# jgaeddert/liquid-usrp

Measured on AMD Instinct MI355X. Metric: complex Msamples/s through multichannelrx, higher is better.
Workload: dtype f32

## Files before the change

liquid-usrp_amd/csrc/ofdmsync.hip:

```cpp
#include "devmath.h"
#include "kernels.h"
#include <utility>

namespace mcrx {

#define WV 64
#ifndef SY_PART
#define SY_PART -1
#endif
#ifndef SY_PROFILE
#define SY_PROFILE 0
#endif
#ifndef H128_EARLY_OUT
#define H128_EARLY_OUT 1
#endif
#ifndef SY_RANK
#define SY_RANK 1
#endif
#ifndef SY_SEG_BURST
#define SY_SEG_BURST 1
#endif
#define SY_PROF(a) (SY_PROFILE && ((a).debug & 2) != 0)
#ifdef MCRX_DEVEL
#define MCRX_DEVEL_ABLATE(a) ((unsigned)(a).debug >> 8 << 6)
// ... 2386 lines not shown
    const int64_t t_ev0 = job->s.cur + (int64_t)job->s.timer - 1;
    const int64_t ws0 = t_ev0 - L + 1 + cb;
    uint32_t dth = uni(job->s.nco_dtheta);
    uint32_t th_ws = uni(job->s.nco_theta_ref + (uint32_t)(ws0 - job->s.nco_t_ref) * job->s.nco_dtheta);
    uint32_t pc = uni(job->s.pilot_count);
    float phi_prime = job->s.phi_prime, p1_prime = job->s.p1_prime;
    int32_t r_ws = (int32_t)uni((uint32_t)(ws0 - a.buf_first));
    const float2 *chb = a.chan + ((size_t)a.chan_off + ch) * MCRX_TILE_S;
    const size_t tstride = (size_t)a.chan_stride * MCRX_TILE_S;
    uint8_t *soft = a.jsoft + (size_t)jj * 8 * c.max_enc_len;
    float2 *syms = reinterpret_cast<float2 *>(a.sarena + job->syms_off);
    const bool soft_mode = c.payload_soft != 0;
    uint32_t nmax = 0;
#pragma unroll
    for (int k = 0; k < FR; k++) {
        const uint32_t v = (uint32_t)__builtin_amdgcn_readlane((int)(active ? nsym : 0u), k * G);
        nmax = v > nmax ? v : nmax;
    }
    const int32_t r_max = (int32_t)(a.end - a.buf_first) - 1;

    auto load_win = [&](int32_t rw, float2 (&x)[E]) {
#pragma unroll
        for (int e = 0; e < E; e++) {
            int32_t r = rw + i + G * e;
            r = r < 0 ? 0 : (r > r_max ? r_max : r);
            x[e] = chb[(size_t)(r >> MCRX_TILE_SH) * tstride + (size_t)(r & (MCRX_TILE_S - 1))];
        }
    };
    float2 cur[E], nxt[E];
    load_win(r_ws, cur);
    uint32_t psi = 0;
    for (uint32_t n = 0; n < nmax; n++) {
        const bool live = active && n < nsym;
        load_win(r_ws + L, nxt);
#pragma unroll
        for (int e = 0; e < E; e++) cur[e] = rot_down(cur[e], u32rev(th_ws + (uint32_t)(i + G * e) * dth));
#pragma unroll
        for (int J = E / 2; J >= 1; J >>= 1) {
#pragma unroll
            for (int e = 0; e < E; e++) {
                if ((e & J) == 0) {
                    const float2 u = cur[e], v = cur[e + J];
                    const float rev = (float)((i + G * e) & (G * J - 1)) * (0.5f / (float)(G * J));
                    cur[e] = cadd(u, v); cur[e + J] = rot_down(csub(u, v), rev);
                }
            }
        }
#define SY_QSTAGE(ST, H)                                                                           \
        if constexpr (H < G) {                                                                     \
            _Pragma("unroll") for (int e = 0; e < E; e++) {                                        \
                const float sx = bfly_leg<H>(cur[e].x, sgc[ST]), sy = bfly_leg<H>(cur[e].y, sgc[ST]);  \
                if (H == 1) cur[e] = make_float2(sx, sy);                                          \
                else cur[e] = make_float2(sx * twc[ST].x - sy * twc[ST].y, sx * twc[ST].y + sy * twc[ST].x); \
            }                                                                                      \
        }
        SY_QSTAGE(0, 32) SY_QSTAGE(1, 16) SY_QSTAGE(2, 8) SY_QSTAGE(3, 4) SY_QSTAGE(4, 2) SY_QSTAGE(5, 1)
#undef SY_QSTAGE
#pragma unroll
        for (int e = 0; e < E; e++) {
            cur[e] = cmul(cur[e], R[e]);
            if (pr[e] >= 0) qpil[16 * g + pr[e]] = cur[e];
        }
        wave_sync_lds();
        float2 P = qpil[16 * g + (i < Mp ? i : 0)];
        uint32_t pi_ = pc + (uint32_t)(i < 16 ? i : 0); pi_ = pi_ >= 255u ? pi_ - 255u : pi_;
        const bool pneg = pseq[pi_ < 255u ? pi_ : 0u] == 0;
        wave_sync_lds();
        if (pneg) { P.x = -P.x; P.y = -P.y; }
        const float v = atan2_fast(P.y, P.x);
        const float prev = dpp_mov<0x111, false>(v, v);
        const float turns = rintf((v - prev) * 0.15915494309189535f);
        const float y = fmaf(-TWO_PI_F, row_scan_fast(turns), v);
        const float p0 = group_total(row_scan_fast(pf0 * y));
        float p1 = group_total(row_scan_fast(pf1 * y));
        pc += (uint32_t)Mp; pc = pc >= 255u ? pc - 255u : pc;
        p1 = 0.3f * p1 + (1.0f - 0.3f) * p1_prime;
        p1_prime = p1;
        const float p0r = p0 * 0.15915494309189535f;
        const bool full = (psi + (uint32_t)Md) * bps <= nbits;
        float2 Z[E];
#pragma unroll
        for (int e = 0; e < E; e++) Z[e] = rot_down(cur[e], fmaf(p1, fxr[e], p0r));
        unsigned long long pending = __ballot(live);
        while (pending) {
            const int src = __builtin_ctzll(pending);
            const uint32_t umod = (uint32_t)__builtin_amdgcn_readlane((int)mod, src), ubps = (uint32_t)__builtin_amdgcn_readlane((int)bps, src);
            const bool sel = live && mod == umod;
            pending &= ~__ballot(sel);
            const uint8_t *unbt = reinterpret_cast<const uint8_t *>(umod == 27 ? qnb16 : qnb64);
#pragma unroll
            for (int e = 0; e < E; e++) {
                const uint32_t idx = psi + (uint32_t)dr[e];
                const bool ok = sel && dr[e] >= 0 && idx < mod_len;
                uint8_t sb[6];
                const unsigned hs = demod_soft(unbt, umod, Z[e], sb);
                if (!soft_mode) {
#pragma unroll
                    for (int kb = 0; kb < 6; kb++) sb[kb] = (uint8_t)(((hs >> ((ubps - 1 - kb) & 7)) & 1) ? 255 : 0);
                }
                if (!ok) continue;
                syms[idx] = Z[e];
                uint8_t *dst = soft + (size_t)idx * ubps;
                if (full) {
                    if (ubps == 2)      *reinterpret_cast<uint16_t *>(dst) = (uint16_t)(sb[0] | (sb[1] << 8));
                    else if (ubps == 1) dst[0] = sb[0];
                    else {
                        *reinterpret_cast<uint16_t *>(dst) = (uint16_t)(sb[0] | (sb[1] << 8));
                        *reinterpret_cast<uint16_t *>(dst + 2) = (uint16_t)(sb[2] | (sb[3] << 8));
                        if (ubps == 6) *reinterpret_cast<uint16_t *>(dst + 4) = (uint16_t)(sb[4] | (sb[5] << 8));
                    }
                } else {
                    for (unsigned kb = 0; kb < ubps; kb++) if (idx * ubps + kb < nbits) dst[kb] = sb[kb];
                }
            }
        }
        psi += (uint32_t)Md;
        float dphi = p0 - phi_prime;
        dphi -= TWO_PI_F * rintf(dphi * 0.15915494309189535f);
        phi_prime = p0;
        const uint32_t dnew = dth + uni((uint32_t)__float2int_rn(dphi * (1e-3f * 683565275.5764316f)));
        th_ws += (uint32_t)(L - cb) * dth + (uint32_t)cb * dnew;
        if (live) dth = dnew;
        r_ws += L;
#pragma unroll
        for (int e = 0; e < E; e++) cur[e] = nxt[e];
    }
    if (i == 0 && active) a.jobs[j].s.nco_dtheta = dth;
}

#include "payload_lean.hpp"

#define DK_T 256
#ifndef DK_FUSED
#define DK_FUSED 1
#endif
#ifndef DK_NT_LOAD
#define DK_NT_LOAD 1
#endif
extern __shared__ __attribute__((aligned(16))) unsigned long long dk_soft[];
#define DKP(e) ((e) ^ (((e) >> 5) & 31u))
__device__ __forceinline__ unsigned il_cols_below(unsigned s0, unsigned len, unsigned Ncol, unsigned rem)
{
    auto span = [&](unsigned a0, unsigned b0) { const unsigned lo = a0 < rem ? a0 : rem, hi = b0 < rem ? b0 : rem; return hi - lo; };
    return (s0 + len <= Ncol) ? span(s0, s0 + len) : span(s0, Ncol) + span(0u, s0 + len - Ncol);
}
__device__ __forceinline__ void divmod_small(unsigned a, unsigned b, unsigned &q, unsigned &r)
{
    q = (unsigned)((float)a * __builtin_amdgcn_rcpf((float)b));
    int rr = (int)a - (int)(q * b);
    if (rr < 0) { q--; rr += (int)b; }
    if (rr >= (int)b) { q++; rr -= (int)b; }
    r = (unsigned)rr;
}
__device__ void il_pass_lds(unsigned n, unsigned Mi, unsigned Ncol, unsigned mask, unsigned dummy)
{
    const unsigned n2 = n / 2, c0 = n / 3;
    unsigned long long m64 = 0;
#pragma unroll
    for (int k = 0; k < 8; k++) if ((mask >> (7 - k)) & 1) m64 |= 0xFFull << (8 * k);
    unsigned R, rem, cnt0 = 0, t0, s1, c0r;
    divmod_small(n2, Ncol, R, rem);
    if (c0 < n2) divmod_small(n2 - c0 + Ncol - 1, Ncol, cnt0, t0);
    divmod_small(c0, Ncol, t0, c0r);
    s1 = c0r + 1; s1 -= s1 >= Ncol ? Ncol : 0u;
    const unsigned sa = s1 < rem ? rem - s1 : 0u, sb = Ncol - (s1 > rem ? s1 : rem), sw = rem < s1 ? rem : s1;
    const unsigned B1 = sa * (R + 1), B2 = B1 + sb * R, B3 = B2 + sw * (R + 1);
    constexpr int UN = 4;
    for (unsigned i0 = threadIdx.x; i0 < n2; i0 += UN * DK_T) {
        unsigned ea[UN], eb[UN];
        unsigned long long va[UN], vb[UN];
#pragma unroll
        for (int u = 0; u < UN; u++) {
            const unsigned i = i0 + u * DK_T;
            const unsigned ip = i - cnt0;
            const bool g1 = ip < B1, g2 = ip < B2, g3 = ip < B3;
            unsigned d = (g1 || (!g2 && g3)) ? R + 1 : R;
            d = d ? d : 1u;
            const unsigned off = g1 ? ip : g2 ? ip - B1 : g3 ? ip - B2 : ip - B3;
            const unsigned lbase = g1 ? 0u : g2 ? sa : g3 ? sa + sb : sa + sb + sw;
            unsigned q, m; divmod_small(off, d, q, m);
            const unsigned len = lbase + q;
            unsigned cm = s1 + len; cm -= cm >= Ncol ? Ncol : 0u;
            const bool first = i < cnt0;
            const unsigned j = first ? i * Ncol + c0 : m * Ncol + cm;
            const bool ok = i < n2 && j < n2 && (first || (len < Ncol && m < Mi));
            ea[u] = ok ? DKP(2 * i) : dummy;
            eb[u] = ok ? DKP(2 * j + 1) : dummy;
            va[u] = dk_soft[ea[u]]; vb[u] = dk_soft[eb[u]];
        }
#pragma unroll
        for (int u = 0; u < UN; u++) {
            dk_soft[ea[u]] = (va[u] & ~m64) | (vb[u] & m64);
            dk_soft[eb[u]] = (vb[u] & ~m64) | (va[u] & m64);
        }
    }
    __syncthreads();
}
__device__ uint32_t crc32_tree(const CodingDev cod, uint32_t tab_off, uint32_t msg_off, uint32_t n)
{
    const uint32_t *lds_tab = reinterpret_cast<const uint32_t *>(reinterpret_cast<const uint8_t *>(dk_soft) + tab_off);
    const uint8_t *p = reinterpret_cast<const uint8_t *>(dk_soft) + msg_off;
    const int r = lane_id();
    uint32_t C = 1, lc = 0;
    while (64u * C < n) { C <<= 1; lc++; }
    const int64_t hi = (int64_t)n - (int64_t)r * C, lo0 = hi - (int64_t)C;
    const int64_t lo = lo0 < 0 ? 0 : lo0;
    const uint32_t rmax = n ? (n + C - 1) / C - 1 : 0;
    uint32_t s = ((uint32_t)r == rmax) ? 0xFFFFFFFFu : 0u;
    for (int64_t i = lo; i < hi; i++) s = (s >> 8) ^ lds_tab[(s ^ p[i]) & 0xff];
#pragma unroll
    for (int k = 0; k < 6; k++) {
        const uint32_t v = (uint32_t)__shfl_down((int)s, 1 << k, WV);
        if ((r & ((2 << k) - 1)) == 0 && r + (1 << k) < WV) {
            const uint32_t *A = cod.crc_zadv + (size_t)(lc + k) * 1024;
            s ^= A[v & 0xff] ^ A[256 + ((v >> 8) & 0xff)] ^ A[512 + ((v >> 16) & 0xff)] ^ A[768 + (v >> 24)];
        }
    }
    return ~(uint32_t)__shfl((int)s, 0, WV);
}
__device__ __forceinline__ void decode_frame(SyncArgs &a, const uint32_t j, uint32_t lds_soft_bytes, uint32_t msg_bytes)
{
    const uint32_t ch = a.jobs[j].ch;
    if (ch >= a.nch || a.jobs[j].arena_off == ~0ull) return;
    const SyncConsts &c = a.c;
    const uint32_t n_msg = a.jobs[j].s.payload_len, crc = a.jobs[j].s.check, fec0 = a.jobs[j].s.fec0, fec1 = a.jobs[j].s.fec1;
    const uint32_t e1 = a.jobs[j].s.enc_len;
    uint8_t *soft = a.jsoft + (size_t)j * 8 * c.max_enc_len;
    const uint32_t crc_len = (crc == 6) ? 4u : 0u, n0 = n_msg + crc_len;
    const bool prof = SY_PROF(a) && j == 7;
    long long tk[8]; int ntk = 0;
#define DK_TICK() if (prof) tk[ntk++] = (long long)__builtin_readcyclecounter();
    DK_TICK()
    const bool lds_path = c.payload_soft && fec0 == 1 && (fec1 == 6 || fec1 == 7 || fec1 == 1) && 8u * e1 <= lds_soft_bytes && !(a.no_fast & 8);
    if (!lds_path) {
        const uint32_t moff = (c.il_off && e1 < c.il_n) ? c.il_off[e1] : ~0u;
        const bool conv_pre = c.payload_soft && fec1 == 11 && a.vit_scratch && moff != ~0u && 8u * e1 <= lds_soft_bytes && !(a.no_fast & 8) &&
                              vf::rows_for(8u * fec_enc_len_d(fec0, n0) + 6u) <= a.vit_rows;
        const bool conv_go = conv_pre;
        if (c.payload_soft && fec1 == 11 && !a.vit_scratch && a.hint && threadIdx.x == 0) a.hint[HINT_K7_SEEN] = 1u;
        if (conv_go) {
            const unsigned long long *g64 = reinterpret_cast<const unsigned long long *>(soft);
            for (uint32_t i = threadIdx.x; i < e1; i += DK_T) dk_soft[DKP(i)] = g64[i];
            __syncthreads();
            const uint4 *mp = reinterpret_cast<const uint4 *>(c.il_map + (size_t)moff * 8);
            const uint8_t *sb = reinterpret_cast<const uint8_t *>(dk_soft);
            unsigned long long *o64 = reinterpret_cast<unsigned long long *>(soft);
            for (uint32_t i = threadIdx.x; i < e1; i += DK_T) {
                const uint4 m = mp[i];
                const uint32_t lo = (uint32_t)sb[m.x & 0xffffu] | ((uint32_t)sb[m.x >> 16] << 8) | ((uint32_t)sb[m.y & 0xffffu] << 16) | ((uint32_t)sb[m.y >> 16] << 24);
                const uint32_t hi = (uint32_t)sb[m.z & 0xffffu] | ((uint32_t)sb[m.z >> 16] << 8) | ((uint32_t)sb[m.w & 0xffffu] << 16) | ((uint32_t)sb[m.w >> 16] << 24);
                o64[i] = (unsigned long long)lo | ((unsigned long long)hi << 32);
            }
        }
        if (threadIdx.x == 0 && a.gen_list) {
            uint32_t *gl = as_global(a.gen_list);
            uint32_t tag = j;
            if (conv_go) {
                tag |= 0x80000000u;
            }
            gl[1u + atomicAdd(gl, 1u)] = tag;
        }
        return;
    }
    if (lds_path) {
        const uint32_t moff_h = (fec1 == 6 && c.il_off && e1 < c.il_n) ? c.il_off[e1] : ~0u;
        const bool fused = DK_FUSED && moff_h != ~0u;
        constexpr int SU = 4;
        const uint2 *mp2 = reinterpret_cast<const uint2 *>(c.il_map + (size_t)(fused ? moff_h : 0u) * 8);
        uint2 pm[SU][3];
        if (fused) {
#pragma unroll
            for (int u = 0; u < SU; u++) {
                const uint32_t i = threadIdx.x + u * DK_T, ii = i < n0 ? i : 0u;
#pragma unroll
                for (int k = 0; k < 3; k++) pm[u][k] = mp2[3u * ii + k];
            }
        }
        const unsigned long long *g64 = reinterpret_cast<const unsigned long long *>(soft);
        for (uint32_t b0 = 0; b0 < e1; b0 += 8 * DK_T) {
            unsigned long long v[8];
#pragma unroll
#if DK_NT_LOAD
            for (int u = 0; u < 8; u++) { const uint32_t i = b0 + u * DK_T + threadIdx.x; v[u] = __builtin_nontemporal_load(g64 + (i < e1 ? i : 0)); }
#else
            for (int u = 0; u < 8; u++) { const uint32_t i = b0 + u * DK_T + threadIdx.x; v[u] = g64[i < e1 ? i : 0]; }
#endif
#pragma unroll
            for (int u = 0; u < 8; u++) { const uint32_t i = b0 + u * DK_T + threadIdx.x; if (i < e1) dk_soft[DKP(i)] = v[u]; }
        }
        __syncthreads();
        DK_TICK()
        unsigned long long *cur = dk_soft;
        uint8_t *msg = reinterpret_cast<uint8_t *>(dk_soft) + 2 * lds_soft_bytes;
        if (fused) {
            const uint8_t *sb = reinterpret_cast<const uint8_t *>(dk_soft);
            for (uint32_t b0 = 0; b0 < n0; b0 += SU * DK_T) {
                if (b0) {
#pragma unroll
                    for (int u = 0; u < SU; u++) {
                        const uint32_t i = b0 + threadIdx.x + u * DK_T, ii = i < n0 ? i : 0u;
#pragma unroll
                        for (int k = 0; k < 3; k++) pm[u][k] = mp2[3u * ii + k];
                    }
                }
#pragma unroll
                for (int u = 0; u < SU; u++) {
                    const uint32_t i = b0 + threadIdx.x + u * DK_T;
                    if (i >= n0) break;
                    uint32_t w[3];
#pragma unroll
                    for (int k = 0; k < 3; k++) {
                        const uint2 m = pm[u][k];
                        w[k] = (uint32_t)sb[m.x & 0xffffu] | ((uint32_t)sb[m.x >> 16] << 8) | ((uint32_t)sb[m.y & 0xffffu] << 16) | ((uint32_t)sb[m.y >> 16] << 24);
                    }
                    msg[i] = (uint8_t)h128_dec_soft_words(w[0], w[1], w[2]);
                }
            }
        } else if (fec1 != 1) {
            const uint32_t moff = (c.il_off && e1 < c.il_n) ? c.il_off[e1] : ~0u;
            if (moff != ~0u) {
                const uint4 *mp = reinterpret_cast<const uint4 *>(c.il_map + (size_t)moff * 8);
                const uint8_t *sb = reinterpret_cast<const uint8_t *>(dk_soft);
                unsigned long long *dst = dk_soft + lds_soft_bytes / 8;
                for (uint32_t i0 = threadIdx.x; i0 < e1; i0 += 8 * DK_T) {
                    uint4 mm[8];
#pragma unroll
                    for (int u = 0; u < 8; u++) { const uint32_t i = i0 + u * DK_T; mm[u] = mp[i < e1 ? i : 0]; }
#pragma unroll
                    for (int u = 0; u < 8; u++) {
                        const uint32_t i = i0 + u * DK_T;
                        if (i >= e1) break;
                        const uint4 m = mm[u];
                        const uint32_t lo = (uint32_t)sb[m.x & 0xffffu] | ((uint32_t)sb[m.x >> 16] << 8) | ((uint32_t)sb[m.y & 0xffffu] << 16) | ((uint32_t)sb[m.y >> 16] << 24);
                        const uint32_t hi = (uint32_t)sb[m.z & 0xffffu] | ((uint32_t)sb[m.z >> 16] << 8) | ((uint32_t)sb[m.w & 0xffffu] << 16) | ((uint32_t)sb[m.w >> 16] << 24);
                        dst[DKP(i)] = (unsigned long long)lo | ((unsigned long long)hi << 32);
                    }
                }
                cur = dst;
                __syncthreads();
            } else {
                unsigned Mi, Ni; il_dims(e1, Mi, Ni);
                const unsigned dummy = 2 * (lds_soft_bytes / 8) + msg_bytes / 8;
                il_pass_lds(e1, Mi, Ni + 8, 0x33, dummy);
                il_pass_lds(e1, Mi, Ni + 4, 0x55, dummy);
                il_pass_lds(e1, Mi, Ni + 2, 0x0f, dummy);
                il_pass_lds(e1, Mi, Ni, 0xff, dummy);
            }
        }
        DK_TICK()
        const uint32_t *w32 = reinterpret_cast<const uint32_t *>(cur);
        auto word = [&](uint32_t w) { return w32[2u * DKP(w >> 1) + (w & 1u)]; };
        auto slice = [&](uint32_t g) -> unsigned {
            const unsigned long long v = cur[DKP(g)];
            unsigned b = 0;
#pragma unroll
            for (int kb = 0; kb < 8; kb++) b = (b << 1) | ((((unsigned)(v >> (8 * kb)) & 0xffu) > 127u) ? 1u : 0u);
            return b;
        };
        if (fused) {
        } else if (fec1 == 6) {
            for (uint32_t i = threadIdx.x; i < n0; i += DK_T) msg[i] = (uint8_t)h128_dec_soft_words(word(3 * i), word(3 * i + 1), word(3 * i + 2));
        } else if (fec1 == 7) {
            const uint32_t G = n0 / 3, rr = n0 % 3;
            for (uint32_t g = threadIdx.x; g < G; g += DK_T) {
                const unsigned s0 = golay_dec_sym((slice(6 * g) << 16) | (slice(6 * g + 1) << 8) | slice(6 * g + 2));
                const unsigned s1 = golay_dec_sym((slice(6 * g + 3) << 16) | (slice(6 * g + 4) << 8) | slice(6 * g + 5));
                msg[3 * g]     = (uint8_t)((s0 >> 4) & 0xff);
                msg[3 * g + 1] = (uint8_t)(((s0 << 4) & 0xf0) | ((s1 >> 8) & 0x0f));
                msg[3 * g + 2] = (uint8_t)(s1 & 0xff);
            }
            if (threadIdx.x < rr) {
                const uint32_t b = 6 * G + 3 * threadIdx.x;
                msg[3 * G + threadIdx.x] = (uint8_t)(golay_dec_sym((slice(b) << 16) | (slice(b + 1) << 8) | slice(b + 2)) & 0xff);
            }
        } else {
            for (uint32_t i = threadIdx.x; i < n0; i += DK_T) msg[i] = (uint8_t)slice(i);
        }
        __syncthreads();
        DK_TICK()
        {
            uint32_t *dst = reinterpret_cast<uint32_t *>(a.arena + a.jobs[j].arena_off);
            const uint32_t *src = reinterpret_cast<const uint32_t *>(msg);
            for (uint32_t i = threadIdx.x; i < (n_msg + 3) / 4; i += DK_T) dst[i] = src[i];
        }
        const bool by_pos = crc_len && c.crc_pos && n_msg >= 4 && n_msg <= c.crc_pos_n;
        if (by_pos) {
            uint32_t acc = 0;
            for (uint32_t i0 = threadIdx.x; i0 < n_msg; i0 += 8 * DK_T) {
                uint32_t t[8];
#pragma unroll
                for (int u = 0; u < 8; u++) {
                    const uint32_t i = i0 + u * DK_T, ii = i < n_msg ? i : n_msg - 1;
                    const uint32_t b = (uint32_t)msg[ii] ^ (ii < 4 ? 0xffu : 0u);
                    t[u] = c.crc_pos[(size_t)(n_msg - 1 - ii) * 256 + b];
                }
#pragma unroll
                for (int u = 0; u < 8; u++) if (i0 + u * DK_T < n_msg) acc ^= t[u];
            }
            acc = wave_xor_u32(acc);
            if ((threadIdx.x & (WV - 1)) == 0) reinterpret_cast<uint32_t *>(dk_soft)[256 + threadIdx.x / WV] = acc;
        }
        reinterpret_cast<uint32_t *>(dk_soft)[threadIdx.x] = c.cod.crc_byte[threadIdx.x];
        __syncthreads();
        if (threadIdx.x >= WV) return;
    }
    bool valid = true;
    if (crc_len) {
        const uint8_t *msg = reinterpret_cast<const uint8_t *>(dk_soft) + 2 * lds_soft_bytes;
        const uint32_t key = ((uint32_t)msg[n_msg] << 24) | ((uint32_t)msg[n_msg + 1] << 16) |
                             ((uint32_t)msg[n_msg + 2] << 8) | (uint32_t)msg[n_msg + 3];
        const bool by_pos = c.crc_pos && n_msg >= 4 && n_msg <= c.crc_pos_n;
        if (by_pos) {
            const uint32_t *part = reinterpret_cast<const uint32_t *>(dk_soft) + 256;
            uint32_t tot = 0;
#pragma unroll
            for (int wv = 0; wv < DK_T / WV; wv++) tot ^= part[wv];
            valid = ~tot == key;
        } else valid = crc32_tree(c.cod, 0u, 2 * lds_soft_bytes, n_msg) == key;
    }
    DK_TICK()
    Walker<1> w(a, ch);
    const PayloadJob job = a.jobs[j];
    if (!w.bind_job(j, job)) return;
    const int64_t nsym = (int64_t)((w.s.mod_len + (uint32_t)c.M_data - 1) / (uint32_t)c.M_data);
    w.emit(w.s.cur + (int64_t)w.s.timer - 1 + (nsym - 1) * (int64_t)c.L, true, valid, false, false);
    DK_TICK()
    if (prof && threadIdx.x == 0) printf("[prof] decode wg7 cycles: stage %lld  passes %lld  h128 %lld  crc %lld  emit %lld\n", tk[1]-tk[0], tk[2]-tk[1], tk[3]-tk[2], tk[4]-tk[3], tk[5]-tk[4]);
#undef DK_TICK
}
__global__ __launch_bounds__(DK_T) void decode_kernel(SyncArgs a, uint32_t lds_soft_bytes, uint32_t msg_bytes)
{
    launder(a);
    uint32_t nl = a.live[0];
    if (nl > a.max_jobs) nl = a.max_jobs;
    for (uint32_t k = blockIdx.x; k < nl; k += gridDim.x) {
        const uint32_t j = a.live[1u + k];
        if (a.dec_phase && j < a.max_jobs) {
            const uint32_t mod = a.jobs[j].s.mod_scheme;
            const bool main_frame = k < a.live_off && (mod == 39 || mod == 40);
            if (main_frame != (a.dec_phase == 1)) continue;
        }
        decode_frame(a, j, lds_soft_bytes, msg_bytes);
        __syncthreads();
    }
}

__global__ __launch_bounds__(WV) __attribute__((amdgpu_num_vgpr(128))) void decode_general_kernel(SyncArgs a)
{
    launder(a);
    __shared__ uint16_t vf_ck[2 * 64 * 64];
    const uint32_t *gl = as_global(a.gen_list);
    uint32_t ng = gl[0];
    if (blockIdx.x == 0 && threadIdx.x == 0 && a.list_hint) a.list_hint[2] = ng;
    if (ng > a.max_jobs) ng = a.max_jobs;
    const SyncConsts &c = a.c;
    const bool have_rows = a.vit_scratch && blockIdx.x < a.vit_waves;
    uint2 *rows = a.vit_scratch + (have_rows ? (size_t)blockIdx.x * a.vit_rows * 64u : 0u);
    for (uint32_t k = blockIdx.x; k < ng; k += gridDim.x) {
        const bool pre_done = (gl[1 + k] & 0x80000000u) != 0;
        const uint32_t j = gl[1 + k] & 0x7fffffffu;
        const uint32_t ch = a.jobs[j].ch;
        if (ch >= a.nch || a.jobs[j].arena_off == ~0ull) continue;
        const uint32_t n_msg = a.jobs[j].s.payload_len, crc = a.jobs[j].s.check, fec0 = a.jobs[j].s.fec0, fec1 = a.jobs[j].s.fec1;
        const size_t tstride = (size_t)c.max_enc_len + 16;
        uint8_t *soft = a.jsoft + (size_t)j * 8 * c.max_enc_len;
        uint8_t *tmpa = a.jtmp + (size_t)j * 2 * tstride, *tmpb = tmpa + tstride;
        if (pre_done) {
            const uint32_t e0 = fec_enc_len_d(fec0, n_msg + ((crc == 6) ? 4u : 0u));
            if (have_rows) vf::decode_frame(soft, e0, tmpa, rows, vf_ck, a.vit_passes);
            else conv27_decode_wave(VitSym{ soft, false }, e0, tmpa, reinterpret_cast<uint16_t *>(tmpb), dk_soft);
            __syncthreads();
        }
        const bool valid = packet_decode(c.cod, c.payload_soft != 0, false, n_msg, crc, fec0, fec1, soft, tmpa, tmpb, dk_soft, MCRX_DEVEL_ABLATE(a), pre_done);
        Walker<1> w(a, ch);
        const PayloadJob job = a.jobs[j];
        if (!w.bind_job(j, job)) continue;
        const int64_t nsym = (int64_t)((w.s.mod_len + (uint32_t)c.M_data - 1) / (uint32_t)c.M_data);
        w.emit(w.s.cur + (int64_t)w.s.timer - 1 + (nsym - 1) * (int64_t)c.L, true, valid, false, true);
        __syncthreads();
    }
}

__global__ __launch_bounds__(WV) void place_jobs_kernel(SyncArgs a)
{
    launder(a);
    if (threadIdx.x != 0) return;
    if (a.gen_list) as_global(a.gen_list)[0] = 0;
    uint32_t nj = *a.njobs;
    if (nj > a.max_jobs) nj = a.max_jobs;
    if (a.njobs_next) *a.njobs_next = 0;
    if (a.qam_next) as_global(a.qam_next)[0] = 0;
    if (a.live_next) as_global(a.live_next)[0] = 0;
    { uint32_t nl = a.live[0]; if (nl > a.max_jobs) a.live[0] = a.max_jobs; }
    if (a.qam_list) {
        uint32_t nq = a.qam_list[0];
        if (nq > a.max_jobs) { nq = a.max_jobs; a.qam_list[0] = nq; }
        if (a.list_hint) a.list_hint[0] = nq;
    }
    if (a.stats) {
        const uint32_t maxenc = a.stats[7];
        a.stats[7] = 0;
        if (a.hint && maxenc) *a.hint = maxenc;
    }
    if (a.walk_hint && a.stats) {
        volatile uint32_t *h = a.walk_hint;
        h[0] = a.stats[0]; h[1] = a.stats[1]; h[2] = a.stats[4]; h[3] = a.stats[5]; h[4] = a.stats[2];
        const uint32_t tot = a.stats[0] + a.stats[1], prev = a.stats[6] <= tot ? a.stats[6] : 0u;
        a.stats[6] = tot;
        h[5] = tot - prev;
        __threadfence_system();
    }
}

__global__ __launch_bounds__(WV) void ilmap_build_kernel(const uint32_t *lens, const uint32_t *offs, uint8_t *lo, uint8_t *hi, uint16_t *map)
{
    const uint32_t e = lens[blockIdx.x];
    const size_t o = (size_t)offs[blockIdx.x] * 8;
    uint8_t *xl = lo + o, *xh = hi + o;
    for (uint32_t i = threadIdx.x; i < 8 * e; i += WV) { xl[i] = (uint8_t)((i >> 3) & 0xff); xh[i] = (uint8_t)((i >> 3) >> 8); }
    __syncthreads();
    deinterleave<true>(xl, e, 4);
    deinterleave<true>(xh, e, 4);
    __syncthreads();
    for (uint32_t i = threadIdx.x; i < 8 * e; i += WV) { const unsigned src = xl[i] | ((unsigned)xh[i] << 8); map[o + i] = (uint16_t)(8u * DKP(src) + (i & 7u)); }
}
hipError_t ilmap_build_launch(const uint32_t *d_lens, const uint32_t *d_offs, uint32_t nlen, uint8_t *d_lo, uint8_t *d_hi, uint16_t *d_map, hipStream_t st)
{
    if (!nlen) return hipSuccess;
    hipLaunchKernelGGL(ilmap_build_kernel, dim3(nlen), dim3(WV), 0, st, d_lens, d_offs, d_lo, d_hi, d_map);
    return hipGetLastError();
}

__global__ void sync_reset_kernel(ChanState *st, uint32_t nch, int64_t cur, float4 *z0, float4 *z1, size_t nz,
                                  uint32_t *nrec, unsigned long long *arena_used, uint32_t *pred_n)
{
    const size_t i = (size_t)blockIdx.x * blockDim.x + threadIdx.x;
    if (i < nz) { const float4 z = make_float4(0.f, 0.f, 0.f, 0.f); if (z0) z0[i] = z; if (z1) z1[i] = z; }
    if (i == 0) { if (nrec) { nrec[0] = 0; nrec[1] = 0; } if (arena_used) { arena_used[0] = 0; arena_used[1] = 0; } }
    if (i >= nch) return;
    if (pred_n) pred_n[i] = 0;
    ChanState z;
    memset(&z, 0, sizeof(z));
    z.state = SY_SEEK; z.cur = cur; z.g0 = 1.0f; z.fstate = FX_HEADER;
    st[i] = z;
}

hipError_t sync_reset_launch(ChanState *st, uint32_t nch, int64_t cur, float2 *hist0, float2 *hist1, size_t hist_n,
                             uint32_t *nrec, unsigned long long *arena_used, uint32_t *pred_n, hipStream_t stream)
{
    const size_t nz = hist_n / 2;
    const size_t n = nz > nch ? nz : nch;
    hipLaunchKernelGGL(sync_reset_kernel, dim3((unsigned)((n + 255) / 256)), dim3(256), 0, stream, st, nch, cur,
                       reinterpret_cast<float4 *>(hist0), reinterpret_cast<float4 *>(hist1), nz, nrec, arena_used, pred_n);
    return hipGetLastError();
}

#endif

enum { SYK_SCOUT = 0, SYK_SPEC = 1, SYK_PAYLOAD_FAST = 2, SYK_PAYLOAD_GENERAL = 3, SYK_LEAN = 4, SYK_TAIL = 5, SYK_WALK = 6 };
hipError_t sy_launch_acq_e1(int what, const SyncArgs &a, unsigned grid, size_t lds, hipStream_t st);
hipError_t sy_launch_acq_e2(int what, const SyncArgs &a, unsigned grid, size_t lds, hipStream_t st);
template <int EE>
static hipError_t sy_launch_acq_width(int what, const SyncArgs &a, unsigned grid, size_t lds, hipStream_t st)
{
    if (what == SYK_SPEC) hipLaunchKernelGGL((sync_spec_kernel<EE>), dim3(grid), dim3(WV), lds, st, a);
    else if (what == SYK_TAIL) hipLaunchKernelGGL((sync_tail_kernel<EE>), dim3(grid), dim3(WV), lds, st, a);
    else hipLaunchKernelGGL((sync_lean_kernel<EE>), dim3(grid), dim3(WV), lds, st, a);
    return hipGetLastError();
}
template <int EE>
static hipError_t sy_launch_width(int what, const SyncArgs &a, unsigned grid, size_t lds, hipStream_t st)
{
    switch (what) {
    case SYK_SCOUT:           hipLaunchKernelGGL((sync_kernel<EE>), dim3(grid), dim3(WV), lds, st, a); break;
    case SYK_SPEC:
        if constexpr (EE == 1) return sy_launch_acq_e1(what, a, grid, lds, st);
        else if constexpr (EE == 2) return sy_launch_acq_e2(what, a, grid, lds, st);
        else hipLaunchKernelGGL((sync_spec_kernel<EE>), dim3(grid), dim3(WV), lds, st, a);
        break;
    case SYK_TAIL:
        if constexpr (EE == 1) return sy_launch_acq_e1(what, a, grid, lds, st);
        else if constexpr (EE == 2) return sy_launch_acq_e2(what, a, grid, lds, st);
        else hipLaunchKernelGGL((sync_kernel<EE>), dim3(grid), dim3(WV), lds, st, a);
// ... 6 lines not shown
    case SYK_WALK:
        if constexpr (EE <= 2) hipLaunchKernelGGL((sync_walk_kernel<EE>), dim3((grid + SY_WALK_WPB - 1) / SY_WALK_WPB), dim3(WV * SY_WALK_WPB), SY_WALK_WPB * SY_LDS_BYTES(EE * WV), st, a);
        else hipLaunchKernelGGL((sync_kernel<EE>), dim3(grid), dim3(WV), lds, st, a);
        break;
    case SYK_PAYLOAD_FAST:    hipLaunchKernelGGL((payload_kernel<EE, true>), dim3(grid), dim3(WV), lds, st, a); break;
    case SYK_PAYLOAD_GENERAL: hipLaunchKernelGGL((payload_kernel<EE, false>), dim3(grid), dim3(WV), lds, st, a); break;
    default: return hipErrorInvalidValue;
    }
    return hipGetLastError();
}
hipError_t sy_launch_e1(int what, const SyncArgs &a, unsigned grid, size_t lds, hipStream_t st);
hipError_t sy_launch_e2(int what, const SyncArgs &a, unsigned grid, size_t lds, hipStream_t st);
hipError_t sy_launch_e4(int what, const SyncArgs &a, unsigned grid, size_t lds, hipStream_t st);
hipError_t sy_launch_e8(int what, const SyncArgs &a, unsigned grid, size_t lds, hipStream_t st);
hipError_t sy_launch_e16(int what, const SyncArgs &a, unsigned grid, size_t lds, hipStream_t st);
#if SY_PART < 0 || SY_PART == 0
hipError_t sy_launch_e1(int what, const SyncArgs &a, unsigned grid, size_t lds, hipStream_t st) { return sy_launch_width<1>(what, a, grid, lds, st); }
hipError_t sy_launch_e2(int what, const SyncArgs &a, unsigned grid, size_t lds, hipStream_t st) { return sy_launch_width<2>(what, a, grid, lds, st); }
#endif
#if SY_PART < 0 || SY_PART == 1
hipError_t sy_launch_e4(int what, const SyncArgs &a, unsigned grid, size_t lds, hipStream_t st) { return sy_launch_width<4>(what, a, grid, lds, st); }
hipError_t sy_launch_e8(int what, const SyncArgs &a, unsigned grid, size_t lds, hipStream_t st) { return sy_launch_width<8>(what, a, grid, lds, st); }
#endif
#if SY_PART < 0 || SY_PART == 2
hipError_t sy_launch_e16(int what, const SyncArgs &a, unsigned grid, size_t lds, hipStream_t st) { return sy_launch_width<16>(what, a, grid, lds, st); }
#endif
#if SY_PART < 0 || SY_PART == 3
hipError_t sy_launch_acq_e1(int what, const SyncArgs &a, unsigned grid, size_t lds, hipStream_t st) { return sy_launch_acq_width<1>(what, a, grid, lds, st); }
hipError_t sy_launch_acq_e2(int what, const SyncArgs &a, unsigned grid, size_t lds, hipStream_t st) { return sy_launch_acq_width<2>(what, a, grid, lds, st); }
#endif

hipError_t acq_lean_launch(const SyncArgs &a, unsigned grid, hipStream_t st);
int acq_lean_waves(const SyncConsts &c);
#if SY_PART < 0 || SY_PART == 4
#include "acq_lean.hpp"
int acq_lean_waves(const SyncConsts &c) { return ((c.M == 64 || c.M == 48) && c.E == 1 && c.M_pilot <= 16 && c.M_pilot >= 1 && c.Nen <= 64) ? ACQ_LEAN_WAVES : 0; }
hipError_t acq_lean_launch(const SyncArgs &a, unsigned grid, hipStream_t st)
{
    if (a.c.M == 48) hipLaunchKernelGGL((acq_lean_kernel<63, 48>), dim3(grid), dim3(WV), 0, st, a);
    else hipLaunchKernelGGL((acq_lean_kernel<63, 64>), dim3(grid), dim3(WV), 0, st, a);
    return hipGetLastError();
}
#endif

hipError_t payload_wide_launch(const SyncArgs &a, unsigned grid, hipStream_t st);
static inline bool payload_wide_takes(const SyncConsts &c) { return (c.E == 2 || c.E == 4) && c.log2M >= 7 && c.M == WV * c.E && c.M_pilot >= 1 && c.M_pilot <= WV; }
#if SY_PART < 0 || SY_PART == 1
#include "payload_wide.hpp"
hipError_t payload_wide_launch(const SyncArgs &a, unsigned grid, hipStream_t st)
{
    if (a.c.E == 2) hipLaunchKernelGGL((payload_wide_kernel<63, 2>), dim3(grid), dim3(WV), 0, st, a);
    else hipLaunchKernelGGL((payload_wide_kernel<63, 4>), dim3(grid), dim3(WV), 0, st, a);
    return hipGetLastError();
}
#endif

#if SY_PART <= 0
static hipError_t sy_launch(int what, const SyncArgs &a0, unsigned grid, size_t lds, hipStream_t st)
{
    SyncArgs a = a0;
    a.vit_off = 0;
    if (what == SYK_SCOUT || what == SYK_TAIL || what == SYK_PAYLOAD_GENERAL || ((what == SYK_LEAN || what == SYK_WALK) && a.c.E > 2)) {
        a.vit_off = (uint32_t)((lds + 15) & ~(size_t)15);
        lds = a.vit_off + (size_t)VIT_B * 8;
    }
    switch (a.c.E) {
    case 1:  return sy_launch_e1(what, a, grid, lds, st);
    case 2:  return sy_launch_e2(what, a, grid, lds, st);
    case 4:  return sy_launch_e4(what, a, grid, lds, st);
    case 8:  return sy_launch_e8(what, a, grid, lds, st);
    case 16: return sy_launch_e16(what, a, grid, lds, st);
    default: return hipErrorInvalidValue;
    }
}

hipError_t sync_launch(const SyncArgs &a, hipStream_t st)
{
    if (a.nch == 0) return hipSuccess;
    if (a.c.M > SY_MAXM) return hipErrorInvalidValue;
    return sy_launch(SYK_SCOUT, a, a.nch, SY_LDS_BYTES(a.c.M), st);
}

hipError_t sync_launch_lean(const SyncArgs &a, hipStream_t st)
{
    if (a.nch == 0) return hipSuccess;
    if (a.c.M > SY_MAXM) return hipErrorInvalidValue;
    return sy_launch(SYK_LEAN, a, a.nch, SY_LDS_BYTES(a.c.M), st);
}

hipError_t sync_launch_walk(const SyncArgs &a, hipStream_t st)
{
    if (a.nch == 0) return hipSuccess;
    if (a.c.M > SY_MAXM) return hipErrorInvalidValue;
    return sy_launch(SYK_WALK, a, a.nch, SY_LDS_BYTES(a.c.M), st);
}

hipError_t sync_launch_tail(const SyncArgs &a, hipStream_t st)
{
    if (a.nch == 0) return hipSuccess;
    return sy_launch(SYK_TAIL, a, a.nch, SY_LDS_BYTES(a.c.M), st);
}

hipError_t sync_launch_spec(const SyncArgs &a, hipStream_t st)
{
    if (a.nch == 0 || a.spec_cap == 0 || a.nseg == 0) return hipSuccess;
    const unsigned grid = a.seg_phase == 1 ? a.nch : a.nch * a.nseg;
    if (acq_lean_waves(a.c) && !a.seg_walker) return acq_lean_launch(a, grid, st);
    return sy_launch(SYK_SPEC, a, grid, SY_LDS_BYTES(a.c.M), st);
}

static uint32_t decode_soft_lds(const SyncArgs &a)
{
    const uint32_t enc_cap = a.enc_hint ? ((a.enc_hint + 127u) & ~127u) : a.c.max_enc_len;
    size_t soft_lds = (size_t)8 * (enc_cap < a.c.max_enc_len ? enc_cap : a.c.max_enc_len);
    if (soft_lds > 56 * 1024) soft_lds = 56 * 1024;
    if (soft_lds < 4096) soft_lds = 4096;
    return (uint32_t)soft_lds;
}

#ifndef SY_REST_FLOOR
#define SY_REST_FLOOR 256u
#endif
#ifndef SY_GEN_FLOOR
#define SY_GEN_FLOOR 128u
#endif
bool sync_payload_splits(const SyncArgs &a)
{
    const bool fast = ((a.c.log2M >= 6 && a.c.M == WV * a.c.E) || (a.c.M == 48 && a.c.E == 1)) && a.c.M_pilot <= WV && !(a.no_fast & 1);
    return a.scout && fast && (a.c.M == WV || a.c.M == 48) && a.c.M_pilot <= 16 && a.payload_fr == 1 && a.payload_lean && !(a.no_fast & 6);
}
hipError_t sync_launch_payload(const SyncArgs &a0, int stage, hipStream_t st)
{
    if (a0.nch == 0 || !a0.scout || a0.max_jobs == 0) return hipSuccess;
    SyncArgs a = a0;
    const unsigned nj = a.max_jobs;
    unsigned ngrid = a.frames_hint == ~0u ? nj : a.frames_hint + a.frames_hint / 4 + 64;
    if (ngrid > nj) ngrid = nj;
    a.live_off = 0;
    const bool fast = ((a.c.log2M >= 6 && a.c.M == WV * a.c.E) || (a.c.M == 48 && a.c.E == 1)) && a.c.M_pilot <= WV && !(a.no_fast & 1);
    const bool m64or48 = a.c.M == WV || a.c.M == 48;
    if (fast && m64or48 && a.c.M_pilot <= 16 && a.payload_fr == 1 && a.payload_lean && !(a.no_fast & 6)) a.live_off = ngrid;
    if (stage == 4 && !a.live_off) return hipSuccess;
    if (!a.live_off) { a.split_rest = 0; a.dec_phase = 0; }
    a.dec_lds_soft = fast ? decode_soft_lds(a) : 0u;
    if (!fast) a.gen_list = nullptr;
    if (stage == 0) {
        hipLaunchKernelGGL(place_jobs_kernel, dim3(1), dim3(WV), 0, st, a);
        return hipGetLastError();
    }
    if (stage == 2) {
        if (!fast) return hipSuccess;
        const size_t soft_lds = a.dec_lds_soft;
        const size_t msg_lds = ((size_t)a.c.max_payload_len + 4 + 15) & ~(size_t)15;
        hipLaunchKernelGGL(decode_kernel, dim3(ngrid), dim3(DK_T), 2 * soft_lds + msg_lds + 16, st, a, (uint32_t)soft_lds, (uint32_t)msg_lds);
        return hipGetLastError();
    }
    if (stage == 3) {
        if (!fast) return hipSuccess;

        unsigned ggrid = a.grid_hint[2] ? (nj < 4096 ? nj : 4096) : SY_GEN_FLOOR;
        if (a.vit_scratch && ggrid > a.vit_waves) ggrid = a.vit_waves;
        hipLaunchKernelGGL(decode_general_kernel, dim3(ggrid), dim3(WV), (size_t)VIT_B * 8, st, a);
        return hipGetLastError();
    }
    const int fr = a.payload_fr;
    if (fast && a.c.M == 48 && a.c.M_pilot <= 16 && fr == 1 && a.payload_lean && !(a.no_fast & 6)) {
        unsigned nq = a.grid_hint[0] == ~0u ? nj : 2u * a.grid_hint[0];
        nq = nq < SY_REST_FLOOR ? SY_REST_FLOOR : (nq > nj ? nj : nq);
        const size_t pad = (size_t)a.payload_lds_pad;
        if (stage != 4) hipLaunchKernelGGL((payload_lean_kernel<63, 48>), dim3(ngrid), dim3(WV), pad, st, a);
        if (stage == 4 || !a.split_rest) hipLaunchKernelGGL((payload_lean_rest_kernel<63, 48>), dim3(a.qam_list ? nq : nj), dim3(WV), pad, st, a);
        return hipGetLastError();
    }
    if (fast && a.c.M == WV && a.c.M_pilot <= 16 && fr > 0 && !(a.no_fast & 6)) {
        if (fr == 4)      hipLaunchKernelGGL(payload_multi_kernel<4>, dim3((nj + 3) / 4), dim3(WV), 0, st, a);
        else if (fr == 2) hipLaunchKernelGGL(payload_multi_kernel<2>, dim3((nj + 1) / 2), dim3(WV), 0, st, a);
        else {
            const int xb = a.payload_xb;
            const size_t pad = (size_t)a.payload_lds_pad;
            if (!a.payload_lean) hipLaunchKernelGGL(payload_multi_kernel<1>, dim3(nj), dim3(WV), pad, st, a);
            else {
                unsigned nq = a.grid_hint[0] == ~0u ? nj : 2u * a.grid_hint[0];
                nq = nq < SY_REST_FLOOR ? SY_REST_FLOOR : (nq > nj ? nj : nq);
#define SY_LEAN(XB) do { if (stage != 4) hipLaunchKernelGGL(payload_lean_kernel<XB>, dim3(ngrid), dim3(WV), pad, st, a); \
                         if (stage == 4 || !a.split_rest) hipLaunchKernelGGL(payload_lean_rest_kernel<XB>, dim3(a.qam_list ? nq : nj), dim3(WV), pad, st, a); } while (0)
                if (xb == 0) SY_LEAN(0);
                else         SY_LEAN(63);
#undef SY_LEAN
            }
        }
        return hipGetLastError();
    }
    if (fast && payload_wide_takes(a.c) && a.payload_lean && a.payload_fr == 1 && !(a.no_fast & 6))
        return payload_wide_launch(a, ngrid, st);
    return sy_launch(fast ? SYK_PAYLOAD_FAST : SYK_PAYLOAD_GENERAL, a, nj, SY_LDS_BYTES(a.c.M), st);
}
#endif

}
```

Measured before the change: 188,500.

## Fuse Golay deinterleave into decode, halve decode LDS, simplify record emit

For Golay-coded frames, the interleaver map is now read directly while slicing and decoding, instead of first writing a deinterleaved copy to a second LDS buffer. This lets the decode kernel request half as much shared memory and adds a launch-bounds occupancy hint. The Walker-based emit is replaced by a lean lane-0 record writer. The change also reduces the fused-path unroll, pins threadIdx in a register, and passes the lane id into the CRC tree. The main risk is that the per-thread gather of map entries adds register pressure, and the new record writer must reproduce exactly what emit did.

Result: no change. 189,100, median of 6 (+0.3%).

```diff
diff --git a/liquid-usrp_amd/csrc/ofdmsync.hip b/liquid-usrp_amd/csrc/ofdmsync.hip
--- a/liquid-usrp_amd/csrc/ofdmsync.hip
+++ b/liquid-usrp_amd/csrc/ofdmsync.hip
@@ -2562,7 +2562,7 @@
     if (rr >= (int)b) { q++; rr -= (int)b; }
     r = (unsigned)rr;
 }
-__device__ void il_pass_lds(unsigned n, unsigned Mi, unsigned Ncol, unsigned mask, unsigned dummy)
+__device__ void il_pass_lds(unsigned n, unsigned Mi, unsigned Ncol, unsigned mask, unsigned dummy, unsigned tid)
 {
     const unsigned n2 = n / 2, c0 = n / 3;
     unsigned long long m64 = 0;
@@ -2576,7 +2576,7 @@
     const unsigned sa = s1 < rem ? rem - s1 : 0u, sb = Ncol - (s1 > rem ? s1 : rem), sw = rem < s1 ? rem : s1;
     const unsigned B1 = sa * (R + 1), B2 = B1 + sb * R, B3 = B2 + sw * (R + 1);
     constexpr int UN = 4;
-    for (unsigned i0 = threadIdx.x; i0 < n2; i0 += UN * DK_T) {
+    for (unsigned i0 = tid; i0 < n2; i0 += UN * DK_T) {
         unsigned ea[UN], eb[UN];
         unsigned long long va[UN], vb[UN];
 #pragma unroll
@@ -2606,11 +2606,10 @@
     }
     __syncthreads();
 }
-__device__ uint32_t crc32_tree(const CodingDev cod, uint32_t tab_off, uint32_t msg_off, uint32_t n)
+__device__ uint32_t crc32_tree(const CodingDev cod, uint32_t tab_off, uint32_t msg_off, uint32_t n, const int r)
 {
     const uint32_t *lds_tab = reinterpret_cast<const uint32_t *>(reinterpret_cast<const uint8_t *>(dk_soft) + tab_off);
     const uint8_t *p = reinterpret_cast<const uint8_t *>(dk_soft) + msg_off;
-    const int r = lane_id();
     uint32_t C = 1, lc = 0;
     while (64u * C < n) { C <<= 1; lc++; }
     const int64_t hi = (int64_t)n - (int64_t)r * C, lo0 = hi - (int64_t)C;
@@ -2628,8 +2627,32 @@
     }
     return ~(uint32_t)__shfl((int)s, 0, WV);
 }
+__device__ __forceinline__ void emit_placed_record(const SyncArgs &a, const uint32_t j, const bool payload_valid, const uint32_t lane)
+{
+    if (lane != 0) return;
+    const SyncConsts &c = a.c;
+    const PayloadJob &job = a.jobs[j];
+    if (job.arena_off == ~0ull) return;
+    const uint32_t idx = job.pad;
+    if (idx >= a.max_rec) { atomicAdd(a.nrec + 1, 1u); return; }
+    const ChanState &s = job.s;
+    const int64_t nsym = (int64_t)((s.mod_len + (uint32_t)c.M_data - 1) / (uint32_t)c.M_data);
+    FrameRec r;
+    r.channel = a.ch_first + job.ch; r.header_valid = s.header_valid; r.payload_valid = payload_valid ? 1 : 0;
+    r.payload_len = s.payload_len;
+    for (int i = 0; i < 8; i++) r.header[i] = (uint8_t)((s.hw[i >> 2] >> (8 * (i & 3))) & 0xffu);
+    r.evm = s.evm; r.rssi = -10.0f * log10f(s.g0);
+    r.cfo = u32rad(s.nco_dtheta) / TWO_PI_F;
+    r.mod_scheme = s.mod_scheme; r.mod_bps = s.bps;
+    r.check = s.check; r.fec0 = s.fec0; r.fec1 = s.fec1;
+    r.num_framesyms = s.mod_len; r.end_sample = s.cur + (int64_t)s.timer - 1 + (nsym - 1) * (int64_t)c.L;
+    r.payload_off = job.arena_off; r.syms_off = job.syms_off;
+    a.rec[idx] = r;
+}
 __device__ __forceinline__ void decode_frame(SyncArgs &a, const uint32_t j, uint32_t lds_soft_bytes, uint32_t msg_bytes)
 {
+    uint32_t tid = threadIdx.x;
+    asm volatile("" : "+v"(tid));
     const uint32_t ch = a.jobs[j].ch;
     if (ch >= a.nch || a.jobs[j].arena_off == ~0ull) return;
     const SyncConsts &c = a.c;
@@ -2647,22 +2670,22 @@
         const bool conv_pre = c.payload_soft && fec1 == 11 && a.vit_scratch && moff != ~0u && 8u * e1 <= lds_soft_bytes && !(a.no_fast & 8) &&
                               vf::rows_for(8u * fec_enc_len_d(fec0, n0) + 6u) <= a.vit_rows;
         const bool conv_go = conv_pre;
-        if (c.payload_soft && fec1 == 11 && !a.vit_scratch && a.hint && threadIdx.x == 0) a.hint[HINT_K7_SEEN] = 1u;
+        if (c.payload_soft && fec1 == 11 && !a.vit_scratch && a.hint && tid == 0) a.hint[HINT_K7_SEEN] = 1u;
         if (conv_go) {
             const unsigned long long *g64 = reinterpret_cast<const unsigned long long *>(soft);
-            for (uint32_t i = threadIdx.x; i < e1; i += DK_T) dk_soft[DKP(i)] = g64[i];
+            for (uint32_t i = tid; i < e1; i += DK_T) dk_soft[DKP(i)] = g64[i];
             __syncthreads();
             const uint4 *mp = reinterpret_cast<const uint4 *>(c.il_map + (size_t)moff * 8);
             const uint8_t *sb = reinterpret_cast<const uint8_t *>(dk_soft);
             unsigned long long *o64 = reinterpret_cast<unsigned long long *>(soft);
-            for (uint32_t i = threadIdx.x; i < e1; i += DK_T) {
+            for (uint32_t i = tid; i < e1; i += DK_T) {
                 const uint4 m = mp[i];
                 const uint32_t lo = (uint32_t)sb[m.x & 0xffffu] | ((uint32_t)sb[m.x >> 16] << 8) | ((uint32_t)sb[m.y & 0xffffu] << 16) | ((uint32_t)sb[m.y >> 16] << 24);
                 const uint32_t hi = (uint32_t)sb[m.z & 0xffffu] | ((uint32_t)sb[m.z >> 16] << 8) | ((uint32_t)sb[m.w & 0xffffu] << 16) | ((uint32_t)sb[m.w >> 16] << 24);
                 o64[i] = (unsigned long long)lo | ((unsigned long long)hi << 32);
             }
         }
-        if (threadIdx.x == 0 && a.gen_list) {
+        if (tid == 0 && a.gen_list) {
             uint32_t *gl = as_global(a.gen_list);
             uint32_t tag = j;
             if (conv_go) {
@@ -2675,13 +2698,13 @@
     if (lds_path) {
         const uint32_t moff_h = (fec1 == 6 && c.il_off && e1 < c.il_n) ? c.il_off[e1] : ~0u;
         const bool fused = DK_FUSED && moff_h != ~0u;
-        constexpr int SU = 4;
+        constexpr int SU = 3;
         const uint2 *mp2 = reinterpret_cast<const uint2 *>(c.il_map + (size_t)(fused ? moff_h : 0u) * 8);
         uint2 pm[SU][3];
         if (fused) {
 #pragma unroll
             for (int u = 0; u < SU; u++) {
-                const uint32_t i = threadIdx.x + u * DK_T, ii = i < n0 ? i : 0u;
+                const uint32_t i = tid + u * DK_T, ii = i < n0 ? i : 0u;
 #pragma unroll
                 for (int k = 0; k < 3; k++) pm[u][k] = mp2[3u * ii + k];
             }
@@ -2691,31 +2714,38 @@
             unsigned long long v[8];
 #pragma unroll
 #if DK_NT_LOAD
-            for (int u = 0; u < 8; u++) { const uint32_t i = b0 + u * DK_T + threadIdx.x; v[u] = __builtin_nontemporal_load(g64 + (i < e1 ? i : 0)); }
+            for (int u = 0; u < 8; u++) { const uint32_t i = b0 + u * DK_T + tid; v[u] = __builtin_nontemporal_load(g64 + (i < e1 ? i : 0)); }
 #else
-            for (int u = 0; u < 8; u++) { const uint32_t i = b0 + u * DK_T + threadIdx.x; v[u] = g64[i < e1 ? i : 0]; }
+            for (int u = 0; u < 8; u++) { const uint32_t i = b0 + u * DK_T + tid; v[u] = g64[i < e1 ? i : 0]; }
 #endif
 #pragma unroll
-            for (int u = 0; u < 8; u++) { const uint32_t i = b0 + u * DK_T + threadIdx.x; if (i < e1) dk_soft[DKP(i)] = v[u]; }
+            for (int u = 0; u < 8; u++) { const uint32_t i = b0 + u * DK_T + tid; if (i < e1) dk_soft[DKP(i)] = v[u]; }
         }
         __syncthreads();
         DK_TICK()
-        unsigned long long *cur = dk_soft;
-        uint8_t *msg = reinterpret_cast<uint8_t *>(dk_soft) + 2 * lds_soft_bytes;
+        uint8_t *msg = reinterpret_cast<uint8_t *>(dk_soft) + lds_soft_bytes;
+        const uint8_t *sb = reinterpret_cast<const uint8_t *>(dk_soft);
+        auto slice_at = [&](const uint4 m) -> unsigned {
+            const unsigned a8[8] = { m.x & 0xffffu, m.x >> 16, m.y & 0xffffu, m.y >> 16, m.z & 0xffffu, m.z >> 16, m.w & 0xffffu, m.w >> 16 };
+            unsigned b = 0;
+#pragma unroll
+            for (int kb = 0; kb < 8; kb++) b = (b << 1) | (sb[a8[kb]] > 127u ? 1u : 0u);
+            return b;
+        };
+        bool done = fused;
         if (fused) {
-            const uint8_t *sb = reinterpret_cast<const uint8_t *>(dk_soft);
             for (uint32_t b0 = 0; b0 < n0; b0 += SU * DK_T) {
                 if (b0) {
 #pragma unroll
                     for (int u = 0; u < SU; u++) {
-                        const uint32_t i = b0 + threadIdx.x + u * DK_T, ii = i < n0 ? i : 0u;
+                        const uint32_t i = b0 + tid + u * DK_T, ii = i < n0 ? i : 0u;
 #pragma unroll
                         for (int k = 0; k < 3; k++) pm[u][k] = mp2[3u * ii + k];
                     }
                 }
 #pragma unroll
                 for (int u = 0; u < SU; u++) {
-                    const uint32_t i = b0 + threadIdx.x + u * DK_T;
+                    const uint32_t i = b0 + tid + u * DK_T;
                     if (i >= n0) break;
                     uint32_t w[3];
 #pragma unroll
@@ -2728,75 +2758,76 @@
             }
         } else if (fec1 != 1) {
             const uint32_t moff = (c.il_off && e1 < c.il_n) ? c.il_off[e1] : ~0u;
-            if (moff != ~0u) {
+            if (moff != ~0u && fec1 == 7) {
                 const uint4 *mp = reinterpret_cast<const uint4 *>(c.il_map + (size_t)moff * 8);
-                const uint8_t *sb = reinterpret_cast<const uint8_t *>(dk_soft);
-                unsigned long long *dst = dk_soft + lds_soft_bytes / 8;
-                for (uint32_t i0 = threadIdx.x; i0 < e1; i0 += 8 * DK_T) {
-                    uint4 mm[8];
-#pragma unroll
-                    for (int u = 0; u < 8; u++) { const uint32_t i = i0 + u * DK_T; mm[u] = mp[i < e1 ? i : 0]; }
-#pragma unroll
-                    for (int u = 0; u < 8; u++) {
-                        const uint32_t i = i0 + u * DK_T;
-                        if (i >= e1) break;
-                        const uint4 m = mm[u];
-                        const uint32_t lo = (uint32_t)sb[m.x & 0xffffu] | ((uint32_t)sb[m.x >> 16] << 8) | ((uint32_t)sb[m.y & 0xffffu] << 16) | ((uint32_t)sb[m.y >> 16] << 24);
-                        const uint32_t hi = (uint32_t)sb[m.z & 0xffffu] | ((uint32_t)sb[m.z >> 16] << 8) | ((uint32_t)sb[m.w & 0xffffu] << 16) | ((uint32_t)sb[m.w >> 16] << 24);
-                        dst[DKP(i)] = (unsigned long long)lo | ((unsigned long long)hi << 32);
-                    }
-                }
-                cur = dst;
-                __syncthreads();
+                const uint32_t G = n0 / 3, rr = n0 % 3;
+                for (uint32_t g0 = 0; g0 < G; g0 += DK_T) {
+                    const uint32_t g = g0 + tid, gg = g < G ? g : 0u;
+                    uint4 mm[6];
+#pragma unroll
+                    for (int u = 0; u < 6; u++) mm[u] = mp[6 * gg + u];
+                    if (g >= G) continue;
+                    const unsigned s0 = golay_dec_sym((slice_at(mm[0]) << 16) | (slice_at(mm[1]) << 8) | slice_at(mm[2]));
+                    const unsigned s1 = golay_dec_sym((slice_at(mm[3]) << 16) | (slice_at(mm[4]) << 8) | slice_at(mm[5]));
+                    msg[3 * g]     = (uint8_t)((s0 >> 4) & 0xff);
+                    msg[3 * g + 1] = (uint8_t)(((s0 << 4) & 0xf0) | ((s1 >> 8) & 0x0f));
+                    msg[3 * g + 2] = (uint8_t)(s1 & 0xff);
+                }
+                if (tid < rr) {
+                    const uint32_t b = 6 * G + 3 * tid;
+                    const uint4 m0 = mp[b], m1 = mp[b + 1], m2 = mp[b + 2];
+                    msg[3 * G + tid] = (uint8_t)(golay_dec_sym((slice_at(m0) << 16) | (slice_at(m1) << 8) | slice_at(m2)) & 0xff);
+                }
+                done = true;
             } else {
                 unsigned Mi, Ni; il_dims(e1, Mi, Ni);
-                const unsigned dummy = 2 * (lds_soft_bytes / 8) + msg_bytes / 8;
-                il_pass_lds(e1, Mi, Ni + 8, 0x33, dummy);
-                il_pass_lds(e1, Mi, Ni + 4, 0x55, dummy);
-                il_pass_lds(e1, Mi, Ni + 2, 0x0f, dummy);
-                il_pass_lds(e1, Mi, Ni, 0xff, dummy);
+                const unsigned dummy = lds_soft_bytes / 8 + msg_bytes / 8;
+                il_pass_lds(e1, Mi, Ni + 8, 0x33, dummy, tid);
+                il_pass_lds(e1, Mi, Ni + 4, 0x55, dummy, tid);
+                il_pass_lds(e1, Mi, Ni + 2, 0x0f, dummy, tid);
+                il_pass_lds(e1, Mi, Ni, 0xff, dummy, tid);
             }
         }
         DK_TICK()
-        const uint32_t *w32 = reinterpret_cast<const uint32_t *>(cur);
+        const uint32_t *w32 = reinterpret_cast<const uint32_t *>(dk_soft);
         auto word = [&](uint32_t w) { return w32[2u * DKP(w >> 1) + (w & 1u)]; };
         auto slice = [&](uint32_t g) -> unsigned {
-            const unsigned long long v = cur[DKP(g)];
+            const unsigned long long v = dk_soft[DKP(g)];
             unsigned b = 0;
 #pragma unroll
             for (int kb = 0; kb < 8; kb++) b = (b << 1) | ((((unsigned)(v >> (8 * kb)) & 0xffu) > 127u) ? 1u : 0u);
             return b;
         };
-        if (fused) {
+        if (done) {
         } else if (fec1 == 6) {
-            for (uint32_t i = threadIdx.x; i < n0; i += DK_T) msg[i] = (uint8_t)h128_dec_soft_words(word(3 * i), word(3 * i + 1), word(3 * i + 2));
+            for (uint32_t i = tid; i < n0; i += DK_T) msg[i] = (uint8_t)h128_dec_soft_words(word(3 * i), word(3 * i + 1), word(3 * i + 2));
         } else if (fec1 == 7) {
             const uint32_t G = n0 / 3, rr = n0 % 3;
-            for (uint32_t g = threadIdx.x; g < G; g += DK_T) {
+            for (uint32_t g = tid; g < G; g += DK_T) {
                 const unsigned s0 = golay_dec_sym((slice(6 * g) << 16) | (slice(6 * g + 1) << 8) | slice(6 * g + 2));
                 const unsigned s1 = golay_dec_sym((slice(6 * g + 3) << 16) | (slice(6 * g + 4) << 8) | slice(6 * g + 5));
                 msg[3 * g]     = (uint8_t)((s0 >> 4) & 0xff);
                 msg[3 * g + 1] = (uint8_t)(((s0 << 4) & 0xf0) | ((s1 >> 8) & 0x0f));
                 msg[3 * g + 2] = (uint8_t)(s1 & 0xff);
             }
-            if (threadIdx.x < rr) {
-                const uint32_t b = 6 * G + 3 * threadIdx.x;
-                msg[3 * G + threadIdx.x] = (uint8_t)(golay_dec_sym((slice(b) << 16) | (slice(b + 1) << 8) | slice(b + 2)) & 0xff);
+            if (tid < rr) {
+                const uint32_t b = 6 * G + 3 * tid;
+                msg[3 * G + tid] = (uint8_t)(golay_dec_sym((slice(b) << 16) | (slice(b + 1) << 8) | slice(b + 2)) & 0xff);
             }
         } else {
-            for (uint32_t i = threadIdx.x; i < n0; i += DK_T) msg[i] = (uint8_t)slice(i);
+            for (uint32_t i = tid; i < n0; i += DK_T) msg[i] = (uint8_t)slice(i);
         }
         __syncthreads();
         DK_TICK()
         {
             uint32_t *dst = reinterpret_cast<uint32_t *>(a.arena + a.jobs[j].arena_off);
             const uint32_t *src = reinterpret_cast<const uint32_t *>(msg);
-            for (uint32_t i = threadIdx.x; i < (n_msg + 3) / 4; i += DK_T) dst[i] = src[i];
+            for (uint32_t i = tid; i < (n_msg + 3) / 4; i += DK_T) dst[i] = src[i];
         }
         const bool by_pos = crc_len && c.crc_pos && n_msg >= 4 && n_msg <= c.crc_pos_n;
         if (by_pos) {
             uint32_t acc = 0;
-            for (uint32_t i0 = threadIdx.x; i0 < n_msg; i0 += 8 * DK_T) {
+            for (uint32_t i0 = tid; i0 < n_msg; i0 += 8 * DK_T) {
                 uint32_t t[8];
 #pragma unroll
                 for (int u = 0; u < 8; u++) {
@@ -2808,15 +2839,15 @@
                 for (int u = 0; u < 8; u++) if (i0 + u * DK_T < n_msg) acc ^= t[u];
             }
             acc = wave_xor_u32(acc);
-            if ((threadIdx.x & (WV - 1)) == 0) reinterpret_cast<uint32_t *>(dk_soft)[256 + threadIdx.x / WV] = acc;
-        }
-        reinterpret_cast<uint32_t *>(dk_soft)[threadIdx.x] = c.cod.crc_byte[threadIdx.x];
+            if ((tid & (WV - 1)) == 0) reinterpret_cast<uint32_t *>(dk_soft)[256 + tid / WV] = acc;
+        }
+        reinterpret_cast<uint32_t *>(dk_soft)[tid] = c.cod.crc_byte[tid];
         __syncthreads();
-        if (threadIdx.x >= WV) return;
+        if (tid >= WV) return;
     }
     bool valid = true;
     if (crc_len) {
-        const uint8_t *msg = reinterpret_cast<const uint8_t *>(dk_soft) + 2 * lds_soft_bytes;
+        const uint8_t *msg = reinterpret_cast<const uint8_t *>(dk_soft) + lds_soft_bytes;
         const uint32_t key = ((uint32_t)msg[n_msg] << 24) | ((uint32_t)msg[n_msg + 1] << 16) |
                              ((uint32_t)msg[n_msg + 2] << 8) | (uint32_t)msg[n_msg + 3];
         const bool by_pos = c.crc_pos && n_msg >= 4 && n_msg <= c.crc_pos_n;
@@ -2826,19 +2857,15 @@
 #pragma unroll
             for (int wv = 0; wv < DK_T / WV; wv++) tot ^= part[wv];
             valid = ~tot == key;
-        } else valid = crc32_tree(c.cod, 0u, 2 * lds_soft_bytes, n_msg) == key;
+        } else valid = crc32_tree(c.cod, 0u, lds_soft_bytes, n_msg, (int)tid) == key;
     }
     DK_TICK()
-    Walker<1> w(a, ch);
-    const PayloadJob job = a.jobs[j];
-    if (!w.bind_job(j, job)) return;
-    const int64_t nsym = (int64_t)((w.s.mod_len + (uint32_t)c.M_data - 1) / (uint32_t)c.M_data);
-    w.emit(w.s.cur + (int64_t)w.s.timer - 1 + (nsym - 1) * (int64_t)c.L, true, valid, false, false);
+    emit_placed_record(a, j, valid, tid);
     DK_TICK()
-    if (prof && threadIdx.x == 0) printf("[prof] decode wg7 cycles: stage %lld  passes %lld  h128 %lld  crc %lld  emit %lld\n", tk[1]-tk[0], tk[2]-tk[1], tk[3]-tk[2], tk[4]-tk[3], tk[5]-tk[4]);
+    if (prof && tid == 0) printf("[prof] decode wg7 cycles: stage %lld  passes %lld  h128 %lld  crc %lld  emit %lld\n", tk[1]-tk[0], tk[2]-tk[1], tk[3]-tk[2], tk[4]-tk[3], tk[5]-tk[4]);
 #undef DK_TICK
 }
-__global__ __launch_bounds__(DK_T) void decode_kernel(SyncArgs a, uint32_t lds_soft_bytes, uint32_t msg_bytes)
+__global__ __launch_bounds__(DK_T, 8) void decode_kernel(SyncArgs a, uint32_t lds_soft_bytes, uint32_t msg_bytes)
 {
     launder(a);
     uint32_t nl = a.live[0];
@@ -3151,7 +3178,7 @@
         if (!fast) return hipSuccess;
         const size_t soft_lds = a.dec_lds_soft;
         const size_t msg_lds = ((size_t)a.c.max_payload_len + 4 + 15) & ~(size_t)15;
-        hipLaunchKernelGGL(decode_kernel, dim3(ngrid), dim3(DK_T), 2 * soft_lds + msg_lds + 16, st, a, (uint32_t)soft_lds, (uint32_t)msg_lds);
+        hipLaunchKernelGGL(decode_kernel, dim3(ngrid), dim3(DK_T), soft_lds + msg_lds + 16, st, a, (uint32_t)soft_lds, (uint32_t)msg_lds);
         return hipGetLastError();
     }
     if (stage == 3) {
```
